# jhhung/kISS

Measured on AMD Instinct MI355X. Metric: bases/sec suffix_sort (chm13v2.0-size synthetic, k=256), higher is better.
Workload: dtype u8; 1 GPU; suffix_sort genome-like synthetic n=3117292070 k=256 (stand-in for chm13v2.0.fa, BASELINE.json configs[1]); PARALLEL_SORTING; text resident in HBM, SA left in HBM; n=3117292070, k=256, seed=2, parallelism=single GPU, lms=905939973, lms_rounds=9, tied_after_round0_item_rounds=184319413, big_segment_item_rounds=72866550, workspace_bytes=80357006484, induce_passes=47

## Files before the change

### include/kiss_hip.h

```cpp
#ifndef KISS_HIP_H
#define KISS_HIP_H

#include <stddef.h>
#include <stdint.h>

#ifdef __cplusplus
extern "C" {
#endif

#define KISS_HIP_VERSION 103

typedef enum kiss_hip_status {
    KISS_HIP_OK = 0,
    KISS_HIP_E_INVALID = -1,
    KISS_HIP_E_NO_DEVICE = -2,
    KISS_HIP_E_HIP = -3,
    KISS_HIP_E_NOMEM = -4,
    KISS_HIP_E_UNSUPPORTED = -5,
    KISS_HIP_E_INTERNAL = -6,
    KISS_HIP_E_IO = -7,
    KISS_HIP_E_DEEP = -8
} kiss_hip_status;

#define KISS_HIP_ALGO_PARALLEL_SORTING 0
// ... 135 lines not shown
};
int kiss_hip_stage_view(kiss_hip_ctx *ctx, int which, void **d_ptr, uint64_t *capacity);
int kiss_hip_stage_reserve(kiss_hip_ctx *ctx, uint64_t lms_capacity);
int kiss_hip_stage_key_hist(kiss_hip_ctx *ctx, const uint64_t *d_keys, uint64_t count, int bits, uint64_t *d_hist,
                            void *stream);
int kiss_hip_stage_partition(kiss_hip_ctx *ctx, const uint64_t *d_keys, const uint32_t *d_pos, uint64_t count, int bits,
                             const uint32_t *splitters, int groups, uint64_t *d_keys_out, uint32_t *d_pos_out,
                             void *stream);
int kiss_hip_stage_sort(kiss_hip_ctx *ctx, const uint64_t *d_keys, const uint32_t *d_pos, uint64_t count, uint64_t n,
                        uint32_t k, uint32_t *d_sorted_out, uint32_t *d_ctx_out, void *stream);
int kiss_hip_stage_induce(kiss_hip_ctx *ctx, uint64_t n, uint32_t k, const uint32_t *d_far_sorted,
                          const uint32_t *d_far_ctx, uint64_t m_far, const uint32_t *d_near_pos, uint64_t near_count,
                          const uint64_t counts12[12], uint32_t *d_SA, void *stream);
int kiss_hip_stage_induce_exact(kiss_hip_ctx *ctx, uint64_t n, uint32_t h0, const uint32_t *d_far_sorted,
                                const uint32_t *d_far_ctx, uint64_t m_far, const uint32_t *d_near_pos, uint64_t near_count,
                                const uint64_t counts12[12], uint32_t *d_SA, void *stream, int *exact_out);
int kiss_hip_stage_refine_exact(kiss_hip_ctx *ctx, uint64_t n, uint32_t h0, uint32_t *d_SA, void *stream);

int kiss_hip_debug_radix_sort(kiss_hip_ctx *ctx, uint64_t *keys, uint32_t *pos, uint64_t count, int key_lo_bit);
int kiss_hip_debug_scan_u32(kiss_hip_ctx *ctx, uint32_t *data, uint64_t count);
int kiss_hip_debug_fail_alloc_over(kiss_hip_ctx *ctx, uint64_t bytes);
int kiss_hip_debug_splitters(const uint64_t *hist, uint64_t bins, int groups, uint32_t *splitters_out,
                             uint64_t *group_counts_out);

typedef struct kiss_hip_fmi_view {
    uint64_t n_sa;
    uint32_t cnt[4];
    uint32_t pri;
    uint32_t sa_intv;
    const uint8_t *bwt;
    const uint32_t *occ1;
    const uint8_t *occ2;
    const uint32_t *sa;
    const uint64_t *b;
    const uint32_t *b_occ;
} kiss_hip_fmi_view;

int kiss_hip_fmi_query_batch_dev(kiss_hip_ctx *ctx, const kiss_hip_fmi_view *fmi, const uint8_t *patterns, uint32_t L,
                                 uint64_t Q, uint32_t *beg, uint32_t *end, uint64_t *hit_count_total,
                                 uint64_t *checksum, uint32_t *offsets, uint64_t *offsets_index,
                                 uint64_t offsets_capacity, void *stream);

int kiss_hip_fmi_build_dev(kiss_hip_ctx *ctx, const uint8_t *d_S, uint64_t n, const uint32_t *d_SA, uint32_t sa_intv,
                           uint8_t *d_bwt, uint32_t *d_occ1, uint8_t *d_occ2, uint32_t *d_sa_sampled, uint64_t *d_b,
                           uint32_t *d_b_occ, uint32_t cnt_out[4], uint32_t *pri_out, void *stream);

// ... 233 lines not shown
```

### kiss_amd/_lib.py

```python
import ctypes
import os

_HERE = os.path.dirname(os.path.abspath(__file__))
LIB_PATH = os.path.join(_HERE, "libkiss_hip.so")
HOOKS_LIB_PATH = os.path.join(_HERE, "libkiss_hip_hooks.so")

KISS_HIP_OK = 0
KISS_HIP_E_INVALID, KISS_HIP_E_NO_DEVICE, KISS_HIP_E_HIP, KISS_HIP_E_NOMEM = -1, -2, -3, -4
KISS_HIP_E_UNSUPPORTED, KISS_HIP_E_INTERNAL, KISS_HIP_E_IO, KISS_HIP_E_DEEP = -5, -6, -7, -8
ALGO_PARALLEL_SORTING = 0
ALGO_PREFIX_DOUBLING = 1
MAX_N = 4294963200
VIEW_LOCAL_KEYS, VIEW_LOCAL_POS, VIEW_PART_KEYS, VIEW_PART_POS, VIEW_SORTED, VIEW_SORTED_CTX = range(6)

KERNEL_CLASSES = [
    "pack", "classify", "radix_hist", "radix_scatter", "scan", "keygather", "flag_compact",
    "place", "induce_count", "induce_scatter", "induce_small", "fm_query", "fm_build", "segrank",
    "group_heads", "isa",
]


class Stats(ctypes.Structure):
    _fields_ = [
        ("n", ctypes.c_uint64), ("m", ctypes.c_uint64), ("k", ctypes.c_uint32), ("depth", ctypes.c_uint32),
# ... 253 lines not shown
    vp, u8p = ctypes.c_void_p, ctypes.c_void_p
    lib.kiss_hip_version.restype = ctypes.c_int
    lib.kiss_hip_strerror.restype = ctypes.c_char_p
    lib.kiss_hip_strerror.argtypes = [ctypes.c_int]
    lib.kiss_hip_device_count.argtypes = [ctypes.POINTER(ctypes.c_int)]
    lib.kiss_hip_ctx_create.argtypes = [ctypes.POINTER(vp), ctypes.c_int, ctypes.c_uint64]
    lib.kiss_hip_ctx_create_sized.argtypes = [ctypes.POINTER(vp), ctypes.c_int, ctypes.c_uint64, ctypes.c_uint64]
    lib.kiss_hip_ctx_release_io_buffers.argtypes = [vp]
    ip = ctypes.POINTER(ctypes.c_int)
    lib.kiss_hip_multi_create.argtypes = [ctypes.POINTER(vp), ip, ctypes.c_int, ctypes.c_uint64]
    lib.kiss_hip_multi_destroy.argtypes = [vp]
    lib.kiss_hip_multi_suffix_sort_dna_u32.argtypes = [vp, vp, ctypes.c_uint64, ctypes.c_uint32, ctypes.c_int, vp]
    lib.kiss_hip_multi_suffix_sort_dna_u32_dev.argtypes = [vp, vp, ctypes.c_uint64, ctypes.c_uint32, ctypes.c_int, vp]
    lib.kiss_hip_multi_get_stats.argtypes = [vp, ctypes.POINTER(MultiStats)]
    lib.kiss_hip_multi_ctx.argtypes = [vp, ctypes.c_int]
    lib.kiss_hip_multi_ctx.restype = vp
    lib.kiss_hip_suffix_sort_dna_u32_multi.argtypes = [vp, ctypes.c_uint64, ctypes.c_uint32, ctypes.c_int, vp, ip, ctypes.c_int]
    lib.kiss_hip_stage_view.argtypes = [vp, ctypes.c_int, ctypes.POINTER(vp), ctypes.POINTER(ctypes.c_uint64)]
    lib.kiss_hip_stage_reserve.argtypes = [vp, ctypes.c_uint64]
    lib.kiss_hip_debug_fail_alloc_over.argtypes = [vp, ctypes.c_uint64]
    lib.kiss_hip_debug_fail_alloc_over.restype = ctypes.c_int
    lib.kiss_hip_debug_splitters.argtypes = [vp, ctypes.c_uint64, ctypes.c_int, vp, vp]
    lib.kiss_hip_debug_splitters.restype = ctypes.c_int
    lib.kiss_hip_ctx_destroy.argtypes = [vp]
    lib.kiss_hip_ctx_set_profiling.argtypes = [vp, ctypes.c_int]
    lib.kiss_hip_ctx_set_profiling_mask.argtypes = [vp, ctypes.c_uint64]
    lib.kiss_hip_last_hip_error.argtypes = [vp, ctypes.POINTER(ctypes.c_char_p)]
    lib.kiss_hip_get_stats.argtypes = [vp, ctypes.POINTER(Stats)]
    lib.kiss_hip_ctx_workspace_bytes.argtypes = [vp, ctypes.POINTER(ctypes.c_uint64)]
    lib.kiss_hip_suffix_sort_dna_u32.argtypes = [u8p, ctypes.c_uint64, ctypes.c_uint32, ctypes.c_int, vp, ctypes.c_int]
    lib.kiss_hip_ctx_suffix_sort_dna_u32.argtypes = [vp, u8p, ctypes.c_uint64, ctypes.c_uint32, ctypes.c_int, vp]
    lib.kiss_hip_ctx_suffix_sort_dna_u32_dev.argtypes = [vp, vp, ctypes.c_uint64, ctypes.c_uint32, ctypes.c_int, vp, vp]
    lib.kiss_hip_ctx_get_stage_outputs.argtypes = [vp, vp, vp, vp]
    lib.kiss_hip_ctx_verify_sa_dev.argtypes = [vp, vp, ctypes.c_uint64, ctypes.c_uint32, vp, ctypes.POINTER(VerifyReport), vp]
    lib.kiss_hip_ctx_verify_sa_dev.restype = ctypes.c_int
    lib.kiss_hip_sa_digest_host.argtypes = [vp, ctypes.c_uint64]
    lib.kiss_hip_sa_digest_host.restype = ctypes.c_uint64
    lib.kiss_hip_fnv1a64_host.argtypes = [vp, ctypes.c_uint64, ctypes.c_uint64]
    lib.kiss_hip_fnv1a64_host.restype = ctypes.c_uint64
    lib.kiss_hip_debug_radix_sort.argtypes = [vp, vp, vp, ctypes.c_uint64, ctypes.c_int]
    lib.kiss_hip_debug_scan_u32.argtypes = [vp, vp, ctypes.c_uint64]
    u64 = ctypes.c_uint64
    lib.kiss_hip_stage_classify.argtypes = [vp, vp, u64, ctypes.c_uint32, u64, u64, ctypes.POINTER(u64 * 13), vp]
    lib.kiss_hip_stage_local_lms.argtypes = [vp, vp, vp, ctypes.POINTER(u64), ctypes.POINTER(u64)]
    lib.kiss_hip_stage_key_hist.argtypes = [vp, vp, u64, ctypes.c_int, vp, vp]
    lib.kiss_hip_stage_partition.argtypes = [vp, vp, vp, u64, ctypes.c_int, vp, ctypes.c_int, vp, vp, vp]
# ... 96 lines not shown
    return lib


def strerror(status):
    return load().kiss_hip_strerror(int(status)).decode()


EXPORTED_SYMBOLS = [
    "kiss_hip_version", "kiss_hip_strerror", "kiss_hip_device_count", "kiss_hip_ctx_create", "kiss_hip_ctx_destroy",
    "kiss_hip_ctx_set_profiling", "kiss_hip_ctx_set_profiling_mask", "kiss_hip_last_hip_error", "kiss_hip_get_stats", "kiss_hip_ctx_workspace_bytes",
    "kiss_hip_suffix_sort_dna_u32", "kiss_hip_ctx_suffix_sort_dna_u32", "kiss_hip_ctx_suffix_sort_dna_u32_dev",
    "kiss_hip_ctx_get_stage_outputs", "kiss_hip_ctx_verify_sa_dev", "kiss_hip_sa_digest_host", "kiss_hip_fnv1a64_host",
    "kiss_hip_fmi_query_batch_dev", "kiss_hip_fmi_build_dev",
    "kiss_hip_debug_radix_sort", "kiss_hip_debug_scan_u32",
    "kiss_hip_stage_classify", "kiss_hip_stage_local_lms", "kiss_hip_stage_key_hist", "kiss_hip_stage_partition",
    "kiss_hip_stage_sort", "kiss_hip_stage_induce", "kiss_hip_stage_induce_exact", "kiss_hip_stage_refine_exact",
    "kiss_hip_fmi_sizes_for", "kiss_hip_fmi_build_host", "kiss_hip_fmi_query_batch_host",
    "kiss_hip_file_size", "kiss_hip_ctx_parse_text_dev", "kiss_hip_ctx_load_text_file", "kiss_hip_copy_to_host",
    "kiss_hip_free_dev", "kiss_hip_alloc_dev", "kiss_hip_suffix_sort_u8", "kiss_hip_ctx_suffix_sort_u8_dev",
    "kiss_hip_ctx_create_sized", "kiss_hip_ctx_release_io_buffers", "kiss_hip_stage_view", "kiss_hip_stage_reserve",
    "kiss_hip_multi_create", "kiss_hip_multi_destroy", "kiss_hip_multi_suffix_sort_dna_u32",
    "kiss_hip_multi_suffix_sort_dna_u32_dev", "kiss_hip_multi_get_stats", "kiss_hip_multi_ctx",
    "kiss_hip_suffix_sort_dna_u32_multi", "kiss_hip_debug_splitters", "kiss_hip_debug_fail_alloc_over",
    "kiss_hip_has_hooks", "kiss_hip_release_cached_contexts", "kiss_hip_get_stats_sized",
    "kiss_hip_fmi_sizes_ex_for", "kiss_hip_fmi_build_ex_dev", "kiss_hip_fmi_query_ex_dev", "kiss_hip_fmi_build_ex_host",
    "kiss_hip_fmi_query_ex_host", "kiss_hip_ctx_lcp_dna_u32_dev", "kiss_hip_ctx_lcp_u8_dev", "kiss_hip_lcp_dna_u32",
    "kiss_hip_lcp_u8", "kiss_hip_fmi_query_mm_dev", "kiss_hip_fmi_query_mm_host",
    "kiss_hip_fmi8_sizes_for", "kiss_hip_fmi8_build_dev", "kiss_hip_fmi8_build_host", "kiss_hip_fmi8_query_dev",
    "kiss_hip_fmi8_query_host", "kiss_hip_fmi_seeds_dev", "kiss_hip_fmi_seeds_host",
    "kiss_hip_fmi_chain_dev", "kiss_hip_fmi_chain_host", "kiss_hip_fmi_align_dev", "kiss_hip_fmi_align_host",
    "kiss_hip_fmi_select_dev", "kiss_hip_fmi_select_host", "kiss_hip_fmi_pair_dev", "kiss_hip_fmi_pair_host",
]
```

### kiss_amd/csrc/api.hip

```cpp
#include "kiss_internal.hpp"
#include <cstdlib>
#include <chrono>
#include <mutex>
#include <cstring>
#include <new>

KTimer::KTimer(kiss_hip_ctx *c, int cls, uint64_t items) : ctx(c), idx(-1)
{
    if (!((ctx->profile_mask >> cls) & 1ull)) return;
    if (ctx->ev_used == ctx->ev_pool.size()) {
        kiss_hip_ctx::Ev e;
        if (hipEventCreate(&e.a) != hipSuccess || hipEventCreate(&e.b) != hipSuccess) return;
        e.cls = 0;
        ctx->ev_pool.push_back(e);
    }
    idx = (int)ctx->ev_used++;
    ctx->ev_pool[idx].cls = cls;
    ctx->stats.launches_kernel[cls]++;
    ctx->stats.items_kernel[cls] += items;
    (void)hipEventRecord(ctx->ev_pool[idx].a, ctx->stream);
}
KTimer::~KTimer()
{
    if (idx >= 0) (void)hipEventRecord(ctx->ev_pool[idx].b, ctx->stream);
// ... 16 lines not shown
}
#ifdef KISS_HIP_HOOKS
static bool env_on(const char *name) { return getenv(name) != nullptr; }
static unsigned long long env_u64(const char *name, unsigned long long dflt)
{
    const char *e = getenv(name);
    return e ? strtoull(e, nullptr, 0) : dflt;
}
void kiss_opts_refresh(kiss_hip_ctx *ctx)
{
    KissOpts o;
    kiss_opts_supported_from_env(o);
    if (const char *e = getenv("KISS_HIP_SYNC_READBACK")) o.sync_readback = atoi(e) != 0;
    o.no_serialize = env_on("KISS_HIP_NO_SERIALIZE");
    o.no_lms_exact = env_on("KISS_HIP_NO_LMS_EXACT");
    o.heads_by_compare = env_on("KISS_HIP_LMS_HEADS_BY_COMPARE");
    o.no_early_out = env_on("KISS_HIP_NO_EARLY_OUT");
    o.no_pivot_rounds = env_on("KISS_HIP_NO_PIVOT_ROUNDS");
    o.pivot_from_round2 = env_on("KISS_HIP_PIVOT_FROM_ROUND2");
    o.pair_keys = env_on("KISS_HIP_PAIR_KEYS");
    o.no_fc0_onepass = env_on("KISS_HIP_NO_FC0_ONEPASS");
    o.no_pair_records = env_on("KISS_HIP_NO_PAIR_RECORDS");
    o.no_small_fused = env_on("KISS_HIP_NO_SMALL_FUSED");
    o.no_class_bytes = env_on("KISS_HIP_NO_CLASS_BYTES");
    o.no_pivot_ctx = env_on("KISS_HIP_NO_PIVOT_CTX");
    o.no_taint = env_on("KISS_HIP_NO_TAINT");
    o.isa_direct = env_on("KISS_HIP_ISA_DIRECT");
    o.no_onesweep = env_on("KISS_HIP_NO_ONESWEEP");
    o.rx_one_tile = env_on("KISS_HIP_RX_ONE_TILE");
    o.merge_lms = env_on("KISS_HIP_MERGE_LMS");
    o.no_small_alphabet = env_on("KISS_HIP_NO_SMALL_ALPHABET");
    o.induce_one_pass = env_on("KISS_HIP_INDUCE_ONE_PASS");
    o.verify = env_on("KISS_HIP_VERIFY");
    o.no_prefault = env_on("KISS_HIP_NO_PREFAULT");
    o.doubling_h0 = (uint32_t)env_u64("KISS_HIP_DOUBLING_H0", 0);
    o.tcap0 = env_u64("KISS_HIP_TCAP0", 0);
    o.pivot_slots = (int)env_u64("KISS_HIP_PIVOT_SLOTS", 3);
    o.small_seg = (uint32_t)env_u64("KISS_HIP_SMALL_SEG", 0);
    o.near_merge_min = (uint32_t)env_u64("KISS_HIP_NEAR_MERGE_MIN", 4096);
    o.induce_small_max = (uint32_t)env_u64("KISS_HIP_INDUCE_SMALL_MAX", 0);
    o.collapse_cap = (uint32_t)env_u64("KISS_HIP_COLLAPSE_CAP", 0);
    o.collapse_n = env_u64("KISS_HIP_COLLAPSE_N", 0);
    o.fm_heavy = (uint32_t)env_u64("KISS_HIP_FM_HEAVY", 0);
    o.fm_light = (uint32_t)env_u64("KISS_HIP_FM_LIGHT", 0);
    o.fm_mm_wave = env_on("KISS_HIP_FM_MM_WAVE");
    o.fm_mm_budget = env_u64("KISS_HIP_FM_MM_BUDGET", 0);
// ... 624 lines not shown
int kiss_hip_last_hip_error(const kiss_hip_ctx *ctx, const char **msg)
{
    if (!ctx) return 0;
    if (msg) *msg = hipGetErrorString((hipError_t)ctx->last_hip_error);
    return ctx->last_hip_error;
}

int kiss_hip_get_stats(const kiss_hip_ctx *ctx, kiss_hip_stats *out)
{
    if (!ctx || !out) return KISS_HIP_E_INVALID;
    *out = ctx->stats;
    return KISS_HIP_OK;
}

int kiss_hip_get_stats_sized(const kiss_hip_ctx *ctx, void *out, uint64_t bytes)
{
    if (!ctx || !out) return KISS_HIP_E_INVALID;
    const uint64_t have = sizeof ctx->stats;
    std::memcpy(out, &ctx->stats, bytes < have ? bytes : have);
    if (bytes > have) std::memset(static_cast<char *>(out) + have, 0, bytes - have);
    return KISS_HIP_OK;
}

int kiss_hip_ctx_release_io_buffers(kiss_hip_ctx *ctx)
{
    if (!ctx) return KISS_HIP_E_INVALID;
    KCHECK(hipSetDevice(ctx->device));
    return kiss_io_release(ctx);
}

int kiss_hip_ctx_workspace_bytes(const kiss_hip_ctx *ctx, uint64_t *bytes)
{
    if (!ctx || !bytes) return KISS_HIP_E_INVALID;
    *bytes = ctx->ws_bytes;
    return KISS_HIP_OK;
}

int kiss_hip_ctx_suffix_sort_dna_u32_dev(kiss_hip_ctx *ctx, const uint8_t *d_S, uint64_t n, uint32_t k, int algo,
                                         uint32_t *d_SA, void *stream)
{
    return sort_dev(ctx, d_S, n, k, algo, d_SA, stream);
}

int kiss_hip_ctx_suffix_sort_dna_u32(kiss_hip_ctx *ctx, const uint8_t *S, uint64_t n, uint32_t k, int algo,
                                     uint32_t *SA)
{
// ... 164 lines not shown
```

### kiss_amd/csrc/kiss_internal.hpp

```cpp
#pragma once
#include <hip/hip_runtime.h>
#include <stdint.h>
#include <stddef.h>
#include <mutex>
#include <vector>
#include "../../include/kiss_hip.h"

struct KissOpts {
    bool debug = false;
    int xfer_threads = 0;
    int prefault_threads = 0;
    bool sync_readback = false;
    bool no_lms_exact = false;
    bool heads_by_compare = false;
    bool no_early_out = false;
    bool no_pivot_rounds = false;
    bool pivot_from_round2 = false;
    bool pair_keys = false;
    bool no_fc0_onepass = false;
    bool no_pair_records = false;
    bool no_small_fused = false;
    bool no_class_bytes = false;
    bool no_pivot_ctx = false;
    bool no_taint = false;
    bool isa_direct = false;
    bool no_onesweep = false;
    bool rx_one_tile = false;
    bool merge_lms = false;
    bool no_small_alphabet = false;
    bool induce_one_pass = false;
    bool verify = false;
    bool no_prefault = false;
    bool no_serialize = false;
    bool lock_launches = false;
    bool sync_launches = false;
    uint32_t doubling_h0 = 0;
    uint64_t tcap0 = 0;
    int pivot_slots = 3;
    uint32_t small_seg = 0;
    uint32_t near_merge_min = 4096;
    uint32_t induce_small_max = 0;
    uint32_t collapse_cap = 0;
    uint64_t collapse_n = 0;
    uint32_t fm_heavy = 0, fm_light = 0;
// ... 174 lines not shown
    uint32_t h_depth = 0;
    bool lms_merged = false;
    int near_form = 0;
    const uint32_t *near_sorted = nullptr;
    const uint32_t *rm_fin = nullptr, *rm_pos = nullptr;
    uint32_t rm_E = 0;

    uint8_t *io_S = nullptr;
    uint32_t *io_SA = nullptr;
    uint64_t io_cap = 0;
    uint32_t *early_host_SA = nullptr;
    hipStream_t early_stream = nullptr;
    std::vector<hipEvent_t> early_events;
    size_t early_used = 0;
    uint64_t early_bytes = 0;
    void *xf_pin[16][2] = {};
    hipEvent_t xf_done[16][2] = {};
    hipStream_t xf_stream[16] = {};
    int xf_ready = 0;

    uint64_t n = 0, m = 0, m_far = 0;
    uint64_t counts[12] = {0};
    kiss_hip_stats stats{};
    uint64_t profile_mask = 0;
    struct Ev { hipEvent_t a, b; int cls; };
    std::vector<Ev> ev_pool;
    size_t ev_used = 0;
};

struct KTimer {
    kiss_hip_ctx *ctx;
    int idx;
    KTimer(kiss_hip_ctx *c, int cls, uint64_t items);
    ~KTimer();
};
void ktimer_collect(kiss_hip_ctx *ctx);

static inline uint64_t div_up(uint64_t a, uint64_t b) { return (a + b - 1) / b; }

int kiss_lms_reserve(kiss_hip_ctx *ctx, uint64_t m_cap, uint64_t t_cap_wanted = 0);
int kiss_tied_reserve(kiss_hip_ctx *ctx, uint64_t t_cap);
int kiss_workspace_ready(kiss_hip_ctx *ctx);
int kiss_need_ctx_words(kiss_hip_ctx *ctx);
int kiss_pack_text(kiss_hip_ctx *ctx, const uint8_t *d_S, uint64_t n);
int kiss_classify(kiss_hip_ctx *ctx, uint64_t n, uint64_t depth , uint64_t win_lo, uint64_t win_hi);
int kiss_readback(kiss_hip_ctx *ctx, const void *d_src, uint32_t nwords);
// ... 112 lines not shown
```

### kiss_amd/csrc/lms_sort.hip

```cpp
#include "kiss_internal.hpp"
#include <cstdio>
#include <cstdlib>
#include <cstring>
#include <ctime>
#include <utility>
#include <vector>

namespace {

constexpr int LS_THREADS = 256;
constexpr uint32_t SMALL_SEG = 64;
constexpr uint32_t LMS_SMALL_SEG = 24;
constexpr int ROUND0_BASES = 20;

__global__ __launch_bounds__(LS_THREADS) void k_gather_keys(const uint64_t *__restrict__ pk, uint64_t n,
                                                           const uint32_t *__restrict__ pos, uint64_t count,
                                                           uint64_t depth_off, uint64_t mask,
                                                           uint64_t *__restrict__ key, const uint32_t *__restrict__ seg,
                                                           const uint32_t *__restrict__ segstart, uint32_t min_len,
                                                           uint32_t max_len)
{
    uint64_t i = (uint64_t)blockIdx.x * LS_THREADS + threadIdx.x;
    if (i >= count) return;
    if (seg) {
        const uint32_t sg = seg[i];
        const uint32_t len = segstart[sg + 1] - segstart[sg];
        if (len < min_len || len > max_len) return;
    }
    uint64_t q = (uint64_t)pos[i] + depth_off;
    uint64_t k = (q < n) ? kiss_key32(pk, q) : 0ull;
    key[i] = k & mask;
}

__device__ __forceinline__ bool deep_less(const uint64_t *__restrict__ pk, uint64_t n, uint64_t pi, uint64_t pj,
                                          uint64_t off, uint64_t depth, bool i_before_j, bool *tied = nullptr)
// ... 511 lines not shown
    key <<= (uint64_t)slotbits * (uint64_t)(slots - used);
    key = (key << 1) | (complete ? 1ull : 0ull);
    keyout[i] = (key << (64 - (slots * slotbits + 1))) | (with_ctx ? (uint64_t)kiss_load_ctx_n(pk, bpos[i], KISS_KEY_CTX_BASES) : 0ull);
}

__global__ __launch_bounds__(LS_THREADS) void k_pivot_heads(const uint64_t *__restrict__ key,
                                                           const uint32_t *__restrict__ seg, uint64_t nbig,
                                                           int complete_bit, uint8_t *__restrict__ heads,
                                                           uint64_t cmp_mask)
{
    const uint64_t i = (uint64_t)blockIdx.x * LS_THREADS + threadIdx.x;
    if (i >= nbig) return;
    const uint64_t k = key[i] & cmp_mask;
    const bool complete = ((k >> complete_bit) & 1ull) != 0;
    const bool same_prev = i > 0 && seg[i] == seg[i - 1] && (key[i - 1] & cmp_mask) == k;
    uint8_t h = 1;
    if (same_prev && !complete) h = 0;
    if (complete && (same_prev || (i + 1 < nbig && seg[i + 1] == seg[i] && (key[i + 1] & cmp_mask) == k))) h |= 2;
    if (complete && same_prev) h |= 4;
    heads[i] = h;
}



constexpr int FC_THREADS = 256;
constexpr int FC_ITEMS = 8;
constexpr int FC_ITEMS_DEFAULT = FC_ITEMS;
constexpr int FC_TILE = FC_THREADS * FC_ITEMS;

constexpr int FC_KEY = 0, FC_KEY_SEG = 1, FC_HEADS = 2;

template <int SRC>
__device__ __forceinline__ void fc_flags(const uint64_t *__restrict__ key, const uint32_t *__restrict__ seg, uint64_t i,
                                         uint64_t count, int cmp_shift, int last_round, bool &surv, bool &shead,
                                         bool *tie = nullptr,
                                         bool *tie_prev = nullptr)
{
    surv = shead = false;
    if (tie) *tie = false;
    if (tie_prev) *tie_prev = false;
    if (i >= count) return;
    bool head, nhead;
    if constexpr (SRC == FC_HEADS) {
        const uint8_t *hb = reinterpret_cast<const uint8_t *>(key);
        head = (i == 0) || hb[i] != 0;
        nhead = (i + 1 == count) || hb[i + 1] != 0;
// ... 888 lines not shown
            b++;
            v >>= 1;
        }
    }
    return b;
}

int read_u64(kiss_hip_ctx *ctx, const void *dptr, uint64_t *out)
{
    KTRY(kiss_readback(ctx, dptr, 2));
    std::memcpy(out, ctx->h_pinned, sizeof(uint64_t));
    return KISS_HIP_OK;
}

}

int kiss_lms_sort(kiss_hip_ctx *ctx, uint64_t n, uint32_t k, uint64_t depth)
{
    (void)k;
    const uint64_t m_far = ctx->m_far;
    ctx->stats.lms_rounds = 0;
    ctx->stats.sort_item_rounds = 0;
    ctx->stats.pair_records = 0;
    if (m_far == 0) return KISS_HIP_OK;
    if (m_far == 1) {
        KCHECK(hipMemcpyAsync(ctx->lms_sorted_far, ctx->lms_pos, sizeof(uint32_t), hipMemcpyDeviceToDevice,
                              ctx->stream));
        KTRY(kiss_zero_u32(ctx, ctx->lms_ctx_far, 1));
        return KISS_HIP_OK;
    }
    uint32_t *d_nbig = ctx->d_small + 8;
    uint64_t *d_total = (uint64_t *)(ctx->d_small + 2);
    const unsigned T = LS_THREADS;
    const bool dbg = ctx->opts.debug;
    const bool pivot_on = !ctx->opts.no_pivot_rounds;
    const bool pivot_r1 = !ctx->opts.pivot_from_round2;
    static const int pivot_den[3] = {4, 7, 11};
    unsigned pivot_rounds_done = 0;
    const int pivot_slots = ctx->opts.pivot_slots >= 1 && ctx->opts.pivot_slots <= 8 ? ctx->opts.pivot_slots : 3;
    const bool no_pair_keys = !ctx->opts.pair_keys;
    const uint32_t small_seg = ctx->opts.small_seg >= 2 && ctx->opts.small_seg <= 4096 ? ctx->opts.small_seg : LMS_SMALL_SEG;
    const bool small_fused = !ctx->opts.no_small_fused && small_seg == LMS_SMALL_SEG;

    uint64_t count = m_far;
    RadixBufs rb;
    rb.first_pos = ctx->lms_pos;
// ... 202 lines not shown
            }
#ifdef KISS_HIP_HOOKS
            if (const char *dump = ctx->opts.dump_pivot[0] ? ctx->opts.dump_pivot : nullptr) {
                std::vector<uint32_t> hp(nbig), hs(nbig), hss(nbigseg + 1);
                std::vector<uint64_t> hk(nbig);
                KCHECK(hipStreamSynchronize(ctx->stream));
                KCHECK(hipMemcpy(hp.data(), ctx->bposA, nbig * 4, hipMemcpyDeviceToHost));
                KCHECK(hipMemcpy(hs.data(), ctx->bsegA, nbig * 4, hipMemcpyDeviceToHost));
                KCHECK(hipMemcpy(hss.data(), bss, (nbigseg + 1) * 4, hipMemcpyDeviceToHost));
                KCHECK(hipMemcpy(hk.data(), ctx->bkeyB, nbig * 8, hipMemcpyDeviceToHost));
                char name[512];
                snprintf(name, sizeof name, "%s.%u", dump, ctx->stats.lms_rounds);
                if (FILE *f = fopen(name, "wb")) {
                    const uint64_t hdr[6] = {nbig, nbigseg, off, depth, (uint64_t)dbits, (uint64_t)slots};
                    fwrite(hdr, 8, 6, f);
                    fwrite(hp.data(), 4, nbig, f);
                    fwrite(hs.data(), 4, nbig, f);
                    fwrite(hss.data(), 4, nbigseg + 1, f);
                    fwrite(hk.data(), 8, nbig, f);
                    fclose(f);
                }
            }
#endif
            RadixBufs pb;
            pb.key[0] = ctx->bkeyB;
            pb.key[1] = ctx->keyB;
            pb.pos[0] = ctx->bposA;
            pb.pos[1] = ctx->bposB;
            pb.seg[0] = ctx->bsegA;
            pb.seg[1] = ctx->bsegB;
            int pres = 0;
            const int sbits = bits_for(nbigseg);
            KTRY(kiss_radix_sort(ctx, pb, nbig, key_lo, sbits, &pres));
            const uint32_t *sseg = sbits ? pb.seg[pres] : ctx->bsegA;
            uint8_t *heads = reinterpret_cast<uint8_t *>(ctx->segB);
            {
                KTimer t(ctx, KISS_HIP_K_FLAG_COMPACT, nbig);
                hipLaunchKernelGGL(k_pivot_heads, dim3(bgrid), dim3(T), 0, ctx->stream, pb.key[pres], sseg, nbig, 64 - kbits,
                                   heads, ~0ull << (64 - kbits));
                KCHECK(hipGetLastError());
            }
            KTRY((fc_count<FC_HEADS>(ctx, reinterpret_cast<const uint64_t *>(heads), nullptr, nbig, 0, 0, d_total)));
            KTRY(fc_read_total(ctx, d_total, &tot));
            KTRY((fc_compact<FC_HEADS, true>(ctx, reinterpret_cast<const uint64_t *>(heads), nullptr, pb.pos[pres], ctx->bslot,
                                            nbig, 0, 0, Pc, Sc, Gc, SSc, ctx->lms_sorted_far, nullptr, nullptr, nullptr, nullptr,
                                            ctx->lms_ctx_far, with_ctx ? pb.key[pres] : (const uint64_t *)nullptr)));
            ctx->stats.big_item_rounds += nbig;
            count = tot >> 32;
            nseg = tot & 0xFFFFFFFFull;
            if (dbg)
                fprintf(stderr, "[kiss_hip]   pivot round: %llu big-segment items in %llu segments -> %llu still tied in %llu "
                                "segments (same depth)\n", (unsigned long long)nbig, (unsigned long long)nbigseg,
                        (unsigned long long)count, (unsigned long long)nseg);
            continue;
        }
        RadixBufs bb;
        uint64_t *H1, *H2;
        if (NE) {
            {
                KTimer t(ctx, KISS_HIP_K_FLAG_COMPACT, nbig);
                hipLaunchKernelGGL(k_pivot_class, dim3(bgrid), dim3(T), 0, ctx->stream, ctx->bkeyA, ctx->bsegA, bss, nbig, F1);
                KCHECK(hipGetLastError());
            }
            KTRY(kiss_scan_u64(ctx, F1, F2, nbig));
            KTimer t(ctx, KISS_HIP_K_FLAG_COMPACT, nbig);
            hipLaunchKernelGGL(k_last_total, dim3(1), dim3(64), 0, ctx->stream, F1, F2, nbig, d_ptot);
            hipLaunchKernelGGL(k_pivot_scatter, dim3(bgrid), dim3(T), 0, ctx->stream, ctx->bkeyA, ctx->bposA, ctx->bsegA, bss,
                               nbig, F1, F2, d_ptot, ctx->bkeyB, ctx->bposB, NE);
            KCHECK(hipGetLastError());
// ... 903 lines not shown
```

### kiss_amd/sorter.py

```python
import ctypes

import numpy as np

from . import _lib

K_UNBOUNDED = 0xFFFFFFFF


_CTX_LIB = {}


def _check(status, where, ctx=None):
    if status != _lib.KISS_HIP_OK:
        detail = ""
        if ctx is not None:
            msg = ctypes.c_char_p()
            lib = _CTX_LIB.get(getattr(ctx, "value", ctx)) or _lib.load()
            code = lib.kiss_hip_last_hip_error(ctx, ctypes.byref(msg))
            if code:
                detail = "hip error %d: %s" % (code, (msg.value or b"").decode())
        raise _lib.KissHipError(status, where, detail)


class Context:
# ... 59 lines not shown
                _check(self._lib.kiss_hip_copy_to_host(out.ctypes.data, ctypes.c_void_p(ptr), n), "kiss_hip_copy_to_host")
        finally:
            self.free_dev(ptr)
        return out

    def set_profiling(self, on, classes=None):
        if on and classes is not None:
            mask = 0
            for c in classes:
                mask |= 1 << _lib.KERNEL_CLASSES.index(c)
            _check(self._lib.kiss_hip_ctx_set_profiling_mask(self._ctx, mask), "kiss_hip_ctx_set_profiling_mask")
        else:
            _check(self._lib.kiss_hip_ctx_set_profiling(self._ctx, 1 if on else 0), "kiss_hip_ctx_set_profiling")

    def workspace_bytes(self):
        v = ctypes.c_uint64()
        _check(self._lib.kiss_hip_ctx_workspace_bytes(self._ctx, ctypes.byref(v)), "kiss_hip_ctx_workspace_bytes")
        return v.value

    def stats(self):
        st = _lib.Stats()
        _check(self._lib.kiss_hip_get_stats(self._ctx, ctypes.byref(st)), "kiss_hip_get_stats")
        return st.as_dict()

    def suffix_sort(self, S, k=256, algo=_lib.ALGO_PARALLEL_SORTING):
        S = np.ascontiguousarray(S, dtype=np.uint8)
        n = S.size
        SA = np.empty(n + 1, dtype=np.uint32)
        _check(self._lib.kiss_hip_ctx_suffix_sort_dna_u32(self._ctx, S.ctypes.data, n, int(k) & 0xFFFFFFFF, int(algo),
                                                          SA.ctypes.data), "kiss_hip_ctx_suffix_sort_dna_u32", self._ctx)
        return SA

    def suffix_sort_host(self, S, SA, k=256, algo=_lib.ALGO_PARALLEL_SORTING):
        assert S.dtype == np.uint8 and SA.dtype == np.uint32 and SA.size == S.size + 1
        assert S.flags["C_CONTIGUOUS"] and SA.flags["C_CONTIGUOUS"]
        _check(self._lib.kiss_hip_ctx_suffix_sort_dna_u32(self._ctx, S.ctypes.data, S.size, int(k) & 0xFFFFFFFF, int(algo),
                                                          SA.ctypes.data), "kiss_hip_ctx_suffix_sort_dna_u32", self._ctx)
        return SA

    def suffix_sort_dev(self, d_S_ptr, n, d_SA_ptr, k=256, algo=_lib.ALGO_PARALLEL_SORTING, stream=None):
        _check(self._lib.kiss_hip_ctx_suffix_sort_dna_u32_dev(self._ctx, ctypes.c_void_p(d_S_ptr), int(n),
                                                              int(k) & 0xFFFFFFFF, int(algo), ctypes.c_void_p(d_SA_ptr),
                                                              ctypes.c_void_p(stream or 0)),
               "kiss_hip_ctx_suffix_sort_dna_u32_dev", self._ctx)

    def verify_sa_dev(self, d_S_ptr, n, d_SA_ptr, k=256, stream=None):
# ... 152 lines not shown
```

Measured before the change: 46.79 billion bases/s.

## Sort mid-size pivot segments with in-LDS bitonic sort instead of global radix

In the pivot round, segments of at most 2048 items are now sorted by a per-workgroup bitonic sort in shared memory. Each key packs the segment id, the key bits and the local index into 64 bits. Only segments longer than that are extracted, radix-sorted globally and written back. This avoids running the multi-pass global radix sort over every big-segment item, at the cost of extra mark, scan and readback steps plus a host sync to size the huge set.

```diff
diff --git a/include/kiss_hip.h b/include/kiss_hip.h
--- a/include/kiss_hip.h
+++ b/include/kiss_hip.h
@@ -181,6 +181,8 @@
 int kiss_hip_debug_fail_alloc_over(kiss_hip_ctx *ctx, uint64_t bytes);
 int kiss_hip_debug_splitters(const uint64_t *hist, uint64_t bins, int groups, uint32_t *splitters_out,
                              uint64_t *group_counts_out);
+
+int kiss_hip_debug_pivot_mid_items(const kiss_hip_ctx *ctx, uint64_t *items);
 
 typedef struct kiss_hip_fmi_view {
     uint64_t n_sa;
diff --git a/kiss_amd/_lib.py b/kiss_amd/_lib.py
--- a/kiss_amd/_lib.py
+++ b/kiss_amd/_lib.py
@@ -299,6 +299,9 @@
     lib.kiss_hip_debug_fail_alloc_over.restype = ctypes.c_int
     lib.kiss_hip_debug_splitters.argtypes = [vp, ctypes.c_uint64, ctypes.c_int, vp, vp]
     lib.kiss_hip_debug_splitters.restype = ctypes.c_int
+    if hasattr(lib, "kiss_hip_debug_pivot_mid_items"):
+        lib.kiss_hip_debug_pivot_mid_items.argtypes = [vp, ctypes.POINTER(ctypes.c_uint64)]
+        lib.kiss_hip_debug_pivot_mid_items.restype = ctypes.c_int
     lib.kiss_hip_ctx_destroy.argtypes = [vp]
     lib.kiss_hip_ctx_set_profiling.argtypes = [vp, ctypes.c_int]
     lib.kiss_hip_ctx_set_profiling_mask.argtypes = [vp, ctypes.c_uint64]
@@ -441,6 +444,7 @@
     "kiss_hip_multi_create", "kiss_hip_multi_destroy", "kiss_hip_multi_suffix_sort_dna_u32",
     "kiss_hip_multi_suffix_sort_dna_u32_dev", "kiss_hip_multi_get_stats", "kiss_hip_multi_ctx",
     "kiss_hip_suffix_sort_dna_u32_multi", "kiss_hip_debug_splitters", "kiss_hip_debug_fail_alloc_over",
+    "kiss_hip_debug_pivot_mid_items",
     "kiss_hip_has_hooks", "kiss_hip_release_cached_contexts", "kiss_hip_get_stats_sized",
     "kiss_hip_fmi_sizes_ex_for", "kiss_hip_fmi_build_ex_dev", "kiss_hip_fmi_query_ex_dev", "kiss_hip_fmi_build_ex_host",
     "kiss_hip_fmi_query_ex_host", "kiss_hip_ctx_lcp_dna_u32_dev", "kiss_hip_ctx_lcp_u8_dev", "kiss_hip_lcp_dna_u32",
diff --git a/kiss_amd/csrc/api.hip b/kiss_amd/csrc/api.hip
--- a/kiss_amd/csrc/api.hip
+++ b/kiss_amd/csrc/api.hip
@@ -62,6 +62,7 @@
     o.no_fc0_onepass = env_on("KISS_HIP_NO_FC0_ONEPASS");
     o.no_pair_records = env_on("KISS_HIP_NO_PAIR_RECORDS");
     o.no_small_fused = env_on("KISS_HIP_NO_SMALL_FUSED");
+    o.no_pivot_mid = env_on("KISS_HIP_NO_PIVOT_MID");
     o.no_class_bytes = env_on("KISS_HIP_NO_CLASS_BYTES");
     o.no_pivot_ctx = env_on("KISS_HIP_NO_PIVOT_CTX");
     o.no_taint = env_on("KISS_HIP_NO_TAINT");
@@ -732,6 +733,13 @@
     return KISS_HIP_OK;
 }
 
+int kiss_hip_debug_pivot_mid_items(const kiss_hip_ctx *ctx, uint64_t *items)
+{
+    if (!ctx || !items) return KISS_HIP_E_INVALID;
+    *items = ctx->pivot_mid_items;
+    return KISS_HIP_OK;
+}
+
 int kiss_hip_ctx_release_io_buffers(kiss_hip_ctx *ctx)
 {
     if (!ctx) return KISS_HIP_E_INVALID;
diff --git a/kiss_amd/csrc/kiss_internal.hpp b/kiss_amd/csrc/kiss_internal.hpp
--- a/kiss_amd/csrc/kiss_internal.hpp
+++ b/kiss_amd/csrc/kiss_internal.hpp
@@ -20,6 +20,7 @@
     bool no_fc0_onepass = false;
     bool no_pair_records = false;
     bool no_small_fused = false;
+    bool no_pivot_mid = false;
     bool no_class_bytes = false;
     bool no_pivot_ctx = false;
     bool no_taint = false;
@@ -240,6 +241,7 @@
     uint64_t n = 0, m = 0, m_far = 0;
     uint64_t counts[12] = {0};
     kiss_hip_stats stats{};
+    uint64_t pivot_mid_items = 0;
     uint64_t profile_mask = 0;
     struct Ev { hipEvent_t a, b; int cls; };
     std::vector<Ev> ev_pool;
diff --git a/kiss_amd/csrc/lms_sort.hip b/kiss_amd/csrc/lms_sort.hip
--- a/kiss_amd/csrc/lms_sort.hip
+++ b/kiss_amd/csrc/lms_sort.hip
@@ -1,4 +1,5 @@
 #include "kiss_internal.hpp"
+#include "pivot_mid.hpp"
 #include <cstdio>
 #include <cstdlib>
 #include <cstring>
@@ -11,6 +12,7 @@
 constexpr int LS_THREADS = 256;
 constexpr uint32_t SMALL_SEG = 64;
 constexpr uint32_t LMS_SMALL_SEG = 24;
+static_assert(PM_MIN_SEG == LMS_SMALL_SEG + 1, "pivot_mid.hpp counts the big segments of a window with this");
 constexpr int ROUND0_BASES = 20;
 
 __global__ __launch_bounds__(LS_THREADS) void k_gather_keys(const uint64_t *__restrict__ pk, uint64_t n,
@@ -568,6 +570,87 @@
 }
 
 
+__global__ __launch_bounds__(PM_THREADS) void k_pivot_mid_sort(uint64_t *key, uint32_t *pos, const uint32_t *__restrict__ bseg,
+                                                               const uint32_t *__restrict__ bss, uint32_t nbig, int key_lo)
+{
+    __shared__ uint64_t sw[PM_WINDOW];
+    __shared__ uint32_t s_lo, s_hi;
+    const int tid = (int)threadIdx.x;
+    const uint32_t w0 = blockIdx.x * PIVOT_MID_MAX;
+    if (tid == 0) {
+        s_lo = ~0u;
+        s_hi = 0;
+    }
+    __syncthreads();
+    uint32_t lo, hi;
+    pm_range(tid, w0, nbig, bseg, bss, lo, hi);
+#pragma unroll
+    for (int d = 32; d >= 1; d >>= 1) {
+        lo = min(lo, (uint32_t)__shfl_xor(lo, d, 64));
+        hi = max(hi, (uint32_t)__shfl_xor(hi, d, 64));
+    }
+    if (lane_id() == 0 && lo < hi) {
+        atomicMin(&s_lo, lo);
+        atomicMax(&s_hi, hi);
+    }
+    __syncthreads();
+    lo = s_lo;
+    hi = s_hi;
+    if (lo >= hi) return;
+    const uint32_t P = pm_pow2(hi - lo);
+    pm_load(tid, lo, hi, P, key_lo, key, bseg, sw);
+    for (uint32_t k2 = 2; k2 <= P; k2 <<= 1)
+        for (uint32_t j = k2 >> 1; j > 0; j >>= 1) {
+            __syncthreads();
+            pm_stage(tid, P, k2, j, sw);
+        }
+    __syncthreads();
+    uint64_t ok[PM_ITEMS];
+    uint32_t op[PM_ITEMS];
+    pm_fetch(tid, lo, hi, sw, key, pos, ok, op);
+    __syncthreads();
+    pm_store(tid, lo, hi, ok, op, key, pos);
+}
+
+__global__ __launch_bounds__(LS_THREADS) void k_pivot_huge_mark(const uint32_t *__restrict__ bss, uint64_t nbigseg,
+                                                               uint64_t *__restrict__ hv)
+{
+    const uint64_t s = (uint64_t)blockIdx.x * LS_THREADS + threadIdx.x;
+    if (s >= nbigseg) return;
+    const uint32_t len = bss[s + 1] - bss[s];
+    hv[s] = len > PIVOT_MID_MAX ? ((uint64_t)len << 32) | 1ull : 0ull;
+}
+
+__global__ __launch_bounds__(LS_THREADS) void k_pivot_huge_extract(const uint64_t *__restrict__ key,
+                                                                  const uint32_t *__restrict__ pos,
+                                                                  const uint32_t *__restrict__ bseg,
+                                                                  const uint32_t *__restrict__ bss, uint64_t nbig,
+                                                                  const uint64_t *__restrict__ hv,
+                                                                  const uint64_t *__restrict__ hex, uint64_t *__restrict__ dkey,
+                                                                  uint32_t *__restrict__ dpos, uint32_t *__restrict__ dseg,
+                                                                  uint32_t *__restrict__ bidx)
+{
+    const uint64_t i = (uint64_t)blockIdx.x * LS_THREADS + threadIdx.x;
+    if (i >= nbig) return;
+    const uint32_t sid = bseg[i];
+    if (!hv[sid]) return;
+    const uint64_t e = hex[sid];
+    const uint32_t kx = (uint32_t)(e >> 32) + ((uint32_t)i - bss[sid]);
+    dkey[kx] = key[i];
+    dpos[kx] = pos[i];
+    dseg[kx] = (uint32_t)e;
+    bidx[kx] = (uint32_t)i;
+}
+
+__global__ __launch_bounds__(LS_THREADS) void k_pivot_size_classes(const uint32_t *__restrict__ bss, uint64_t nbigseg,
+                                                                  unsigned long long *__restrict__ cls)
+{
+    const uint64_t s = (uint64_t)blockIdx.x * LS_THREADS + threadIdx.x;
+    if (s >= nbigseg) return;
+    const uint32_t len = bss[s + 1] - bss[s];
+    const int c = len <= 1024 ? 0 : (len <= 2048 ? 1 : (len <= 4096 ? 2 : (len <= 8192 ? 3 : 4)));
+    atomicAdd(cls + c, (unsigned long long)len);
+}
 
 constexpr int FC_THREADS = 256;
 constexpr int FC_ITEMS = 8;
@@ -1502,6 +1585,7 @@
     ctx->stats.lms_rounds = 0;
     ctx->stats.sort_item_rounds = 0;
     ctx->stats.pair_records = 0;
+    ctx->pivot_mid_items = 0;
     if (m_far == 0) return KISS_HIP_OK;
     if (m_far == 1) {
         KCHECK(hipMemcpyAsync(ctx->lms_sorted_far, ctx->lms_pos, sizeof(uint32_t), hipMemcpyDeviceToDevice,
@@ -1750,29 +1834,99 @@
                 }
             }
 #endif
-            RadixBufs pb;
-            pb.key[0] = ctx->bkeyB;
-            pb.key[1] = ctx->keyB;
-            pb.pos[0] = ctx->bposA;
-            pb.pos[1] = ctx->bposB;
-            pb.seg[0] = ctx->bsegA;
-            pb.seg[1] = ctx->bsegB;
-            int pres = 0;
-            const int sbits = bits_for(nbigseg);
-            KTRY(kiss_radix_sort(ctx, pb, nbig, key_lo, sbits, &pres));
-            const uint32_t *sseg = sbits ? pb.seg[pres] : ctx->bsegA;
+            const uint64_t *skey;
+            const uint32_t *spos, *sseg;
+            uint64_t nhuge = nbig, nhugeseg = nbigseg;
+            uint64_t *const hv = F1, *const hex = F1 + nbigseg;
+            const int sort_lo = 64 - kbits;
+            const bool mid_on = !ctx->opts.no_pivot_mid && small_seg >= LMS_SMALL_SEG && pm_fields_fit(sort_lo) &&
+                                2 * nbigseg <= ctx->t_cap && nbig <= ctx->m_cap;
+            if (dbg) {
+                unsigned long long *cls = reinterpret_cast<unsigned long long *>(ctx->d_small + 32);
+                KTRY(kiss_zero_u32(ctx, cls, 10));
+                hipLaunchKernelGGL(k_pivot_size_classes, dim3((unsigned)div_up(nbigseg, T)), dim3(T), 0, ctx->stream, bss, nbigseg, cls);
+                KCHECK(hipGetLastError());
+                KTRY(kiss_readback(ctx, cls, 10));
+                uint64_t c[5];
+                std::memcpy(c, ctx->h_pinned, sizeof c);
+                fprintf(stderr, "[kiss_hip]   pivot round: big-segment items by segment size: <=1024 %llu, <=2048 %llu, <=4096 %llu, "
+                                "<=8192 %llu, larger %llu\n", (unsigned long long)c[0], (unsigned long long)c[1],
+                        (unsigned long long)c[2], (unsigned long long)c[3], (unsigned long long)c[4]);
+            }
+            if (mid_on) {
+                {
+                    KTimer t(ctx, KISS_HIP_K_FLAG_COMPACT, nbigseg);
+                    hipLaunchKernelGGL(k_pivot_huge_mark, dim3((unsigned)div_up(nbigseg, T)), dim3(T), 0, ctx->stream, bss, nbigseg, hv);
+                    KCHECK(hipGetLastError());
+                }
+                KTRY(kiss_scan_u64(ctx, hv, hex, nbigseg));
+                hipLaunchKernelGGL(k_last_total, dim3(1), dim3(64), 0, ctx->stream, hv, hex, nbigseg, d_total);
+                uint64_t ht;
+                KTRY(read_u64(ctx, d_total, &ht));
+                nhuge = ht >> 32;
+                nhugeseg = ht & 0xFFFFFFFFull;
+                if (nhuge > nbig || nhugeseg > nbigseg) return KINTERNAL();
+            }
+            if (nhuge < nbig) {
+                {
+                    KTimer t(ctx, KISS_HIP_K_RADIX_SCATTER, nbig - nhuge);
+                    hipLaunchKernelGGL(k_pivot_mid_sort, dim3((unsigned)div_up(nbig, PIVOT_MID_MAX)), dim3(PM_THREADS), 0, ctx->stream,
+                                       ctx->bkeyB, ctx->bposA, ctx->bsegA, bss, (uint32_t)nbig, sort_lo);
+                    KCHECK(hipGetLastError());
+                }
+                if (nhuge) {
+                    RadixBufs hb;
+                    hb.key[0] = ctx->bkeyA;
+                    hb.key[1] = ctx->keyB;
+                    hb.pos[0] = ctx->bposB;
+                    hb.pos[1] = ctx->lmsP;
+                    hb.seg[0] = ctx->bsegB;
+                    hb.seg[1] = ctx->segB;
+                    uint32_t *bidx = ctx->lmsC;
+                    {
+                        KTimer t(ctx, KISS_HIP_K_FLAG_COMPACT, nbig);
+                        hipLaunchKernelGGL(k_pivot_huge_extract, dim3(bgrid), dim3(T), 0, ctx->stream, ctx->bkeyB, ctx->bposA,
+                                           ctx->bsegA, bss, nbig, hv, hex, hb.key[0], hb.pos[0], hb.seg[0], bidx);
+                        KCHECK(hipGetLastError());
+                    }
+                    int hres = 0;
+                    KTRY(kiss_radix_sort(ctx, hb, nhuge, key_lo, bits_for(nhugeseg), &hres));
+                    KTimer t(ctx, KISS_HIP_K_FLAG_COMPACT, nhuge);
+                    hipLaunchKernelGGL(k_big_writeback, dim3((unsigned)div_up(nhuge, T)), dim3(T), 0, ctx->stream, hb.key[hres],
+                                       hb.pos[hres], bidx, nhuge, ctx->bkeyB, ctx->bposA);
+                    KCHECK(hipGetLastError());
+                }
+                ctx->pivot_mid_items += nbig - nhuge;
+                skey = ctx->bkeyB;
+                spos = ctx->bposA;
+                sseg = ctx->bsegA;
+            } else {
+                RadixBufs pb;
+                pb.key[0] = ctx->bkeyB;
+                pb.key[1] = ctx->keyB;
+                pb.pos[0] = ctx->bposA;
+                pb.pos[1] = ctx->bposB;
+                pb.seg[0] = ctx->bsegA;
+                pb.seg[1] = ctx->bsegB;
+                int pres = 0;
+                const int sbits = bits_for(nbigseg);
+                KTRY(kiss_radix_sort(ctx, pb, nbig, key_lo, sbits, &pres));
+                skey = pb.key[pres];
+                spos = pb.pos[pres];
+                sseg = sbits ? pb.seg[pres] : ctx->bsegA;
+            }
             uint8_t *heads = reinterpret_cast<uint8_t *>(ctx->segB);
             {
                 KTimer t(ctx, KISS_HIP_K_FLAG_COMPACT, nbig);
-                hipLaunchKernelGGL(k_pivot_heads, dim3(bgrid), dim3(T), 0, ctx->stream, pb.key[pres], sseg, nbig, 64 - kbits,
+                hipLaunchKernelGGL(k_pivot_heads, dim3(bgrid), dim3(T), 0, ctx->stream, skey, sseg, nbig, 64 - kbits,
                                    heads, ~0ull << (64 - kbits));
                 KCHECK(hipGetLastError());
             }
             KTRY((fc_count<FC_HEADS>(ctx, reinterpret_cast<const uint64_t *>(heads), nullptr, nbig, 0, 0, d_total)));
             KTRY(fc_read_total(ctx, d_total, &tot));
-            KTRY((fc_compact<FC_HEADS, true>(ctx, reinterpret_cast<const uint64_t *>(heads), nullptr, pb.pos[pres], ctx->bslot,
+            KTRY((fc_compact<FC_HEADS, true>(ctx, reinterpret_cast<const uint64_t *>(heads), nullptr, spos, ctx->bslot,
                                             nbig, 0, 0, Pc, Sc, Gc, SSc, ctx->lms_sorted_far, nullptr, nullptr, nullptr, nullptr,
-                                            ctx->lms_ctx_far, with_ctx ? pb.key[pres] : (const uint64_t *)nullptr)));
+                                            ctx->lms_ctx_far, with_ctx ? skey : (const uint64_t *)nullptr)));
             ctx->stats.big_item_rounds += nbig;
             count = tot >> 32;
             nseg = tot & 0xFFFFFFFFull;
diff --git a/kiss_amd/csrc/pivot_mid.hpp b/kiss_amd/csrc/pivot_mid.hpp
--- /dev/null
+++ b/kiss_amd/csrc/pivot_mid.hpp
@@ -0,0 +1,106 @@
+#pragma once
+#include <stdint.h>
+
+#ifdef __HIPCC__
+#define PM_HD __host__ __device__ __forceinline__
+#else
+#define PM_HD inline
+#endif
+
+#ifndef KISS_PIVOT_MID_MAX
+#define KISS_PIVOT_MID_MAX 2048
+#endif
+constexpr uint32_t PIVOT_MID_MAX = KISS_PIVOT_MID_MAX;
+constexpr uint32_t PM_MIN_SEG = 25;
+constexpr int PM_ITEMS = 8;
+constexpr uint32_t PM_WINDOW = 2 * PIVOT_MID_MAX;
+constexpr int PM_THREADS = (int)(PM_WINDOW / PM_ITEMS);
+constexpr int pm_bits_for(uint32_t count) { return count <= 1 ? 0 : 1 + pm_bits_for((count + 1) / 2); }
+constexpr int PM_IDX_BITS = pm_bits_for(PM_WINDOW);
+constexpr int PM_SEG_BITS = pm_bits_for(PIVOT_MID_MAX / PM_MIN_SEG + 2);
+static_assert((PIVOT_MID_MAX & (PIVOT_MID_MAX - 1)) == 0 && PIVOT_MID_MAX >= 512 && PIVOT_MID_MAX <= 4096,
+              "PIVOT_MID_MAX: a power of two, 64 to 1024 threads per workgroup");
+static_assert((1u << PM_IDX_BITS) == PM_WINDOW, "index field");
+
+PM_HD bool pm_fields_fit(int key_lo) { return key_lo > 0 && key_lo < 64 && PM_SEG_BITS + (64 - key_lo) + PM_IDX_BITS <= 64; }
+
+PM_HD bool pm_owned(uint32_t a, uint32_t b, uint32_t w0) { return a >= w0 && a - w0 < PIVOT_MID_MAX && b - a <= PIVOT_MID_MAX; }
+
+PM_HD void pm_range(int tid, uint32_t w0, uint32_t nbig, const uint32_t *bseg, const uint32_t *bss, uint32_t &lo, uint32_t &hi)
+{
+    lo = ~0u;
+    hi = 0;
+    for (int e = 0; e < PM_ITEMS; e++) {
+        const uint32_t off = (uint32_t)e * PM_THREADS + (uint32_t)tid;
+        if (off >= nbig - w0) break;
+        const uint32_t i = w0 + off, sid = bseg[i];
+        if (pm_owned(bss[sid], bss[sid + 1], w0)) {
+            if (i < lo) lo = i;
+            if (i + 1 > hi) hi = i + 1;
+        }
+    }
+}
+
+PM_HD uint32_t pm_pow2(uint32_t m)
+{
+    uint32_t p = 64;
+    while (p < m) p <<= 1;
+    return p;
+}
+
+PM_HD void pm_load(int tid, uint32_t lo, uint32_t hi, uint32_t P, int key_lo, const uint64_t *key, const uint32_t *bseg,
+                   uint64_t *sw)
+{
+    const uint32_t m = hi - lo, sid_lo = bseg[lo];
+    const int kb = 64 - key_lo;
+    for (int e = 0; e < PM_ITEMS; e++) {
+        const uint32_t j = (uint32_t)e * PM_THREADS + (uint32_t)tid;
+        if (j >= P) break;
+        uint64_t w = ~0ull;
+        if (j < m)
+            w = ((uint64_t)(bseg[lo + j] - sid_lo) << (kb + PM_IDX_BITS)) | ((key[lo + j] >> key_lo) << PM_IDX_BITS) | (uint64_t)j;
+        sw[j] = w;
+    }
+}
+
+PM_HD void pm_stage(int tid, uint32_t P, uint32_t k2, uint32_t j, uint64_t *sw)
+{
+    for (uint32_t t = (uint32_t)tid; t < P / 2; t += PM_THREADS) {
+        const uint32_t i = ((t & ~(j - 1)) << 1) | (t & (j - 1)), l = i | j;
+        const bool up = (i & k2) == 0;
+        const uint64_t a = sw[i], b = sw[l];
+        if ((a > b) == up) {
+            sw[i] = b;
+            sw[l] = a;
+        }
+    }
+}
+
+PM_HD void pm_fetch(int tid, uint32_t lo, uint32_t hi, const uint64_t *sw, const uint64_t *key, const uint32_t *pos,
+                    uint64_t ok[PM_ITEMS], uint32_t op[PM_ITEMS])
+{
+    const uint32_t m = hi - lo;
+    for (int e = 0; e < PM_ITEMS; e++) {
+        const uint32_t j = (uint32_t)e * PM_THREADS + (uint32_t)tid;
+        ok[e] = 0;
+        op[e] = 0;
+        if (j < m) {
+            const uint32_t src = lo + (uint32_t)(sw[j] & (uint64_t)(PM_WINDOW - 1));
+            ok[e] = key[src];
+            op[e] = pos[src];
+        }
+    }
+}
+
+PM_HD void pm_store(int tid, uint32_t lo, uint32_t hi, const uint64_t ok[PM_ITEMS], const uint32_t op[PM_ITEMS], uint64_t *key,
+                    uint32_t *pos)
+{
+    const uint32_t m = hi - lo;
+    for (int e = 0; e < PM_ITEMS; e++) {
+        const uint32_t j = (uint32_t)e * PM_THREADS + (uint32_t)tid;
+        if (j < m) {
+            key[lo + j] = ok[e];
+            pos[lo + j] = op[e];
+        }
+    }
+}
diff --git a/kiss_amd/sorter.py b/kiss_amd/sorter.py
--- a/kiss_amd/sorter.py
+++ b/kiss_amd/sorter.py
@@ -105,6 +105,11 @@
         st = _lib.Stats()
         _check(self._lib.kiss_hip_get_stats(self._ctx, ctypes.byref(st)), "kiss_hip_get_stats")
         return st.as_dict()
+
+    def pivot_mid_items(self):
+        v = ctypes.c_uint64()
+        _check(self._lib.kiss_hip_debug_pivot_mid_items(self._ctx, ctypes.byref(v)), "kiss_hip_debug_pivot_mid_items")
+        return v.value
 
     def suffix_sort(self, S, k=256, algo=_lib.ALGO_PARALLEL_SORTING):
         S = np.ascontiguousarray(S, dtype=np.uint8)
```

Result: no change. 47.08 billion bases/s (median of 6 runs) (+0.6%).
